# leok7v/sqz

Measured on AMD Instinct MI355X. Metric: encode MB/s + decode MB/s, 32KB window, batched blocks, 1/2/4/8 MI355X, higher is better.
Workload: dtype u8; 1 GPU; 4096 x 262144 B Zipf(s=1) byte blocks, window 2^15, one independent stream per block (BASELINE.json configs[2]); total_blocks=4096, blocks_per_gpu=4096, block_bytes=262144, win_bits=15, parallelism=1 rank; the N>1 runs shard this same batch (strong scaling), finder=index, device=AMD Radeon Graphics (gfx950:sramecc+:xnack-)

## Files before the change

### sqz_amd/csrc/lz77_index.hip

```cpp
#include "sqz_device.h"
#include "sqz_kernels.h"

namespace sqzk {

constexpr int kSharedGiveUp = 8;
constexpr int kXcds = 8;
constexpr int kSortThreads = 1024;
constexpr int kSortWaves = kSortThreads / kWave;

constexpr int kSortTile = 4 * kSortThreads;

constexpr int kSortBins = 1024;
constexpr int kSortCntRow = kSortBins + 2;
struct SortLds {
    uint32_t elem[kSortTile];
    uint16_t dig[kSortTile];
    uint16_t cnt[kSortWaves][kSortCntRow];
    uint32_t gbase[3][kSortBins];
    uint32_t delta[kSortBins];
    uint32_t wtot[kSortWaves];
};

struct __attribute__((packed)) U32u { uint32_t v; };

__device__ __forceinline__ uint32_t load_u32_unaligned(const uint8_t* p) {
    return reinterpret_cast<const U32u*>(p)->v;
}

__device__ __forceinline__ uint64_t peers_of(uint32_t digit, bool valid, int bits) {
    const uint64_t all = __ballot(valid);
    uint32_t lo = (uint32_t)all, hi = (uint32_t)(all >> 32);
#pragma unroll
    for (int bit = 0; bit < 10; bit++) {
        if (bit < bits) {
            const uint32_t mine = (uint32_t)((int32_t)(digit << (31 - bit)) >> 31);
            const uint64_t m = __ballot(mine != 0u);
            lo &= ~((uint32_t)m ^ mine);
            hi &= ~((uint32_t)(m >> 32) ^ mine);
        }
    }
    return ((uint64_t)hi << 32) | lo;
}

__device__ __forceinline__ uint32_t lanes_below(uint64_t mask) {
    return __builtin_amdgcn_mbcnt_hi((uint32_t)(mask >> 32),
                                     __builtin_amdgcn_mbcnt_lo((uint32_t)mask, 0u));
}

__device__ __forceinline__ uint32_t sort_key(const uint8_t* src, uint64_t bytes, uint32_t k) {
    return (uint64_t)k + 4 <= bytes ? (__builtin_bswap32(load_u32_unaligned(src + k)) >> 8)
                                    : (((uint32_t)src[k] << 16) | ((uint32_t)src[k + 1] << 8) | (uint32_t)src[k + 2]);
}

typedef uint32_t __attribute__((may_alias)) SortCntPair;

struct SortSec {
#ifdef SQZ_STATS
    uint64_t t[8] = {0, 0, 0, 0, 0, 0, 0, 0};
    uint64_t last = 0;
#endif
};
#ifdef SQZ_STATS
#define SORT_SEC(s, k) { const uint64_t n_ = __builtin_readcyclecounter(); (s).t[k] += n_ - (s).last; (s).last = n_; }
#define SORT_SEC_LOADS(s, k) { asm volatile("s_waitcnt vmcnt(0)" ::: "memory"); SORT_SEC(s, k) }
#else
#define SORT_SEC(s, k)
#define SORT_SEC_LOADS(s, k)
#endif

template <int kBits, bool kSmall>
__device__ __forceinline__ void sort_pass(SortLds& lds, const int pass, const uint8_t* __restrict__ src,
                                          const uint64_t bytes, const uint32_t count, const bool carry,
                                          const uint32_t* __restrict__ from, uint32_t* __restrict__ to, SortSec& sec) {
    constexpr int kDigits = 1 << kBits;
    constexpr int kTpd = kSortThreads / kDigits;
    constexpr int kWpt = kSortWaves / kTpd;
    const int tid = threadIdx.x;
    const int lane = tid & (kWave - 1);
    const int wave = __builtin_amdgcn_readfirstlane(tid >> 6);
    const bool first = kSmall ? kBits == 10 : pass == 0;
    uint32_t* const gbase = lds.gbase[pass];

    auto fetch = [&](uint32_t tile, uint32_t (&raw)[4]) {
#pragma unroll
        for (int j = 0; j < 4; j++) {
            const uint32_t k = tile + (uint32_t)(wave * 256 + j * kWave + lane);
            if (first) {
                const uint32_t last = (uint32_t)(bytes - 4);
                raw[j] = load_u32_unaligned(src + (k < last ? k : last));
            } else {
                raw[j] = from[k < count ? k : count - 1u];
            }
        }
    };
    auto key_from = [&](uint32_t raw, uint32_t k) {
        const uint32_t be = __builtin_bswap32(raw);
        return (uint64_t)k + 4 <= bytes ? be >> 8 : be & 0x00FFFFFFu;
    };
    auto decode = [&](uint32_t tile, const uint32_t (&raw)[4], uint32_t (&elem)[4], uint32_t (&digit)[4], bool (&valid)[4]) {
#pragma unroll
        for (int j = 0; j < 4; j++) {
            const uint32_t k = tile + (uint32_t)(wave * 256 + j * kWave + lane);
            valid[j] = k < count;
            const uint32_t pos = valid[j] ? (first ? k : raw[j]) : 0u;
            digit[j] = 0; elem[j] = pos;
            if (!valid[j]) { continue; }
            if (kSmall) {
                if (first) {
                    const uint32_t key = key_from(raw[j], k);
                    digit[j] = key & 0x3FFu;
                    elem[j] = pos | ((key >> 10) << 18);
                } else if (pass == 1) {
                    digit[j] = (pos >> 18) & 0x7Fu;
                } else {
                    digit[j] = pos >> 25;
                    elem[j] = pos & 0x3FFFFu;
                }
            } else if (first) {
                digit[j] = key_from(raw[j], k) & 0xFFu;
            } else if (pass == 1) {
                const uint32_t w = (uint32_t)src[pos] | ((uint32_t)src[pos + 1] << 8);
                digit[j] = w >> 8;
                if (carry) { elem[j] = pos | ((w & 0xFFu) << 24); }
            } else {
                digit[j] = carry ? (pos >> 24) : (uint32_t)src[pos];
                if (carry) { elem[j] = pos & 0x00FFFFFFu; }
            }
        }
    };

    uint32_t ahead[4], elem[4], digit[4], wrank[4];
    bool valid[4];
    fetch(0u, ahead);
    decode(0u, ahead, elem, digit, valid);
    SORT_SEC_LOADS(sec, 1)
    for (uint32_t tile = 0; tile < count; tile += (uint32_t)kSortTile) {
        const uint32_t n_tile = count - tile < (uint32_t)kSortTile ? count - tile : (uint32_t)kSortTile;
        fetch(tile + (uint32_t)kSortTile, ahead);
        {
            SortCntPair* const row = reinterpret_cast<SortCntPair*>(lds.cnt[wave]);
            for (int d = lane; d < kDigits / 2; d += kWave) { row[d] = 0u; }
        }
#pragma unroll
        for (int j = 0; j < 4; j++) {
            const uint64_t peers = peers_of(digit[j], valid[j], kBits);
            const uint32_t rank = lanes_below(peers);
            wrank[j] = valid[j] ? (uint32_t)lds.cnt[wave][digit[j]] + rank : 0u;
            __builtin_amdgcn_wave_barrier();
            if (valid[j] && rank == 0) {
                lds.cnt[wave][digit[j]] = (uint16_t)(lds.cnt[wave][digit[j]] + (uint32_t)__builtin_popcountll(peers));
            }
            __builtin_amdgcn_wave_barrier();
        }
        lds_barrier();
        SORT_SEC(sec, 2)
        const int sd = tid / kTpd;
        const int sw = (tid % kTpd) * kWpt;
        uint32_t c[kWpt], sum = 0;
#pragma unroll
        for (int i = 0; i < kWpt; i++) { c[i] = lds.cnt[sw + i][sd]; sum += c[i]; }
        const uint32_t incl = wave_scan(sum);
        if (lane == kWave - 1) { lds.wtot[wave] = incl; }
        lds_barrier();
        SORT_SEC(sec, 3)
        uint32_t at = wave_scan(lane < wave ? lds.wtot[lane] : 0u);
        at = (uint32_t)__builtin_amdgcn_readlane((int)at, kWave - 1) + incl - sum;
        const uint32_t run = at;
#pragma unroll
        for (int i = 0; i < kWpt; i++) { lds.cnt[sw + i][sd] = (uint16_t)at; at += c[i]; }
        const uint32_t run_end = kTpd > 1 ? (uint32_t)__shfl((int)at, lane | (kTpd - 1)) : at;
        if (tid % kTpd == 0) {
            const uint32_t g = gbase[sd];
            lds.delta[sd] = g - run;
            gbase[sd] = g + (run_end - run);
        }
        lds_barrier();
        SORT_SEC(sec, 4)
#pragma unroll
        for (int j = 0; j < 4; j++) {
            if (valid[j]) {
                const uint32_t slot = (uint32_t)lds.cnt[wave][digit[j]] + wrank[j];
                if (slot < (uint32_t)kSortTile) {
                    lds.elem[slot] = elem[j];
                    lds.dig[slot] = (uint16_t)digit[j];
                }
            }
        }
        lds_barrier();
        SORT_SEC(sec, 5)
#pragma unroll
        for (int j = 0; j < 4; j++) {
            const uint32_t slot = (uint32_t)(j * kSortThreads + tid);
            const uint32_t s = slot < n_tile ? slot : n_tile - 1u;
            const uint32_t dest = s + lds.delta[lds.dig[s]];
            to[dest < count ? dest : count - 1u] = lds.elem[s];
        }
        SORT_SEC(sec, 6)
        decode(tile + (uint32_t)kSortTile, ahead, elem, digit, valid);
        SORT_SEC_LOADS(sec, 1)
    }
    __threadfence_block();
    __syncthreads();
}

__global__ __launch_bounds__(kSortThreads)
void index_sort_kernel(const uint8_t* __restrict__ in,
                       const uint64_t* __restrict__ in_off,
                       uint32_t n_blocks,
                       uint32_t* __restrict__ buf_a,
                       uint32_t* __restrict__ buf_b,
                       uint64_t slots) {
    __shared__ SortLds lds;
    const uint32_t b = blockIdx.x;
    if (b >= n_blocks || in_off[b + 1] > slots) { return; }
    const int tid = threadIdx.x;
    const int lane = tid & (kWave - 1);
    const int wave = __builtin_amdgcn_readfirstlane(tid >> 6);

    const uint8_t* src = in + in_off[b];
    const uint64_t bytes = in_off[b + 1] - in_off[b];
    if (bytes < 3) { return; }
    const uint32_t count = (uint32_t)(bytes - 2);
    uint32_t* const pa = buf_a + in_off[b];
    uint32_t* const pb = buf_b + in_off[b];
    if (bytes == 3) {
        if (tid == 0) { pa[0] = 0u; }
        return;
    }
    const bool small = bytes <= (1u << 18);
    const bool carry = bytes <= (1u << 24);
    const int w0 = small ? 10 : 8, w1 = small ? 7 : 8, w2 = small ? 7 : 8;
    const int s1 = w0, s2 = w0 + w1;
    const uint32_t m0 = (1u << w0) - 1u, m1 = (1u << w1) - 1u;
    SortSec sec;
#ifdef SQZ_STATS
    sec.last = __builtin_readcyclecounter();
    const uint64_t sec_begin = sec.last;
#endif
    for (int d = tid; d < 3 * kSortBins; d += kSortThreads) { (&lds.gbase[0][0])[d] = 0; }
    __syncthreads();
    auto count_key = [&](uint32_t key) {
        atomicAdd(&lds.gbase[0][key & m0], 1u);
        atomicAdd(&lds.gbase[1][(key >> s1) & m1], 1u);
        atomicAdd(&lds.gbase[2][key >> s2], 1u);
    };
    const uint32_t quads = bytes >= 8 ? (uint32_t)((bytes - 8) / 4) + 1u : 0u;
    if ((uint32_t)tid < quads) {
        uint32_t lo = load_u32_unaligned(src + 4u * (uint32_t)tid), hi = load_u32_unaligned(src + 4u * (uint32_t)tid + 4u);
        for (uint32_t q = (uint32_t)tid; q < quads; q += (uint32_t)kSortThreads) {
            const uint64_t eight = ((uint64_t)hi << 32) | lo;
            const uint32_t nq = q + (uint32_t)kSortThreads < quads ? q + (uint32_t)kSortThreads : q;
            lo = load_u32_unaligned(src + 4u * nq); hi = load_u32_unaligned(src + 4u * nq + 4u);
#pragma unroll
            for (int j = 0; j < 4; j++) { count_key(__builtin_bswap32((uint32_t)(eight >> (8 * j))) >> 8); }
        }
    }
    for (uint32_t k = 4u * quads + (uint32_t)tid; k < count; k += (uint32_t)kSortThreads) { count_key(sort_key(src, bytes, k)); }
    __syncthreads();
    if (wave < 3) {
        uint32_t* const g = lds.gbase[wave];
        const int per = (1 << (wave == 0 ? w0 : wave == 1 ? w1 : w2)) / kWave;
        uint32_t sum = 0;
        for (int j = 0; j < per; j++) { sum += g[per * lane + j]; }
        uint32_t excl = wave_scan(sum) - sum;
        for (int j = 0; j < per; j++) { const uint32_t v = g[per * lane + j]; g[per * lane + j] = excl; excl += v; }
    }
    __syncthreads();
    SORT_SEC(sec, 0)

    if (small) {
        sort_pass<10, true>(lds, 0, src, bytes, count, carry, pb, pa, sec);
        for (int pass = 1; pass < 3; pass++) {
            sort_pass<7, true>(lds, pass, src, bytes, count, carry, pass == 1 ? pa : pb, pass == 1 ? pb : pa, sec);
        }
    } else {
        for (int pass = 0; pass < 3; pass++) {
            sort_pass<8, false>(lds, pass, src, bytes, count, carry, pass == 1 ? pa : pb, pass == 1 ? pb : pa, sec);
        }
    }
#ifdef SQZ_STATS
    if (tid == 0 && b == 1) {
        printf("sort block 1: cycles %llu: hist %llu; tiles: loads %llu rank %llu scan_a %llu scan_b %llu place %llu copy_out %llu\n",
               (unsigned long long)(sec.last - sec_begin), (unsigned long long)sec.t[0], (unsigned long long)sec.t[1],
               (unsigned long long)sec.t[2], (unsigned long long)sec.t[3], (unsigned long long)sec.t[4],
               (unsigned long long)sec.t[5], (unsigned long long)sec.t[6]);
    }
#endif
}

__global__ __launch_bounds__(256)
void index_match_kernel(const uint8_t* __restrict__ in,
                        const uint64_t* __restrict__ in_off,
                        uint32_t n_blocks, uint32_t window,
                        const uint32_t* __restrict__ sorted,
                        uint32_t* __restrict__ match, uint32_t groups, uint64_t slots) {
    const uint32_t xcd = blockIdx.x % (uint32_t)kXcds;
    const uint32_t local = blockIdx.x / (uint32_t)kXcds;
    const uint32_t b = (local / groups) * (uint32_t)kXcds + xcd;
    const uint32_t group = local % groups;
    if (b >= n_blocks || in_off[b + 1] > slots) { return; }
    const uint8_t* src = in + in_off[b];
    const uint64_t bytes = in_off[b + 1] - in_off[b];
    if (bytes < 3) { return; }
    const uint32_t n = (uint32_t)bytes;
    const uint32_t count = n - 2;
    const uint32_t* S = sorted + in_off[b];
    uint32_t* M = match + in_off[b];

    const int lane = (int)(threadIdx.x & (kWave - 1));
    const uint32_t pages = (count + (uint32_t)kWave - 1u) / (uint32_t)kWave;
    const uint32_t waves = groups * (blockDim.x / (uint32_t)kWave);
    const uint32_t per_wave = (pages + waves - 1u) / waves;
    const uint32_t wave_id = group * (blockDim.x / (uint32_t)kWave) + (threadIdx.x - (uint32_t)lane) / (uint32_t)kWave;
    const uint32_t page_lo = wave_id * per_wave;
    const uint32_t page_hi = page_lo + per_wave < pages ? page_lo + per_wave : pages;
    auto load16 = [&](uint32_t at, uint32_t& w0, uint32_t& w1, uint32_t& w2, uint32_t& w3) {
        if (at + 16 <= n) {
            w0 = load_u32_unaligned(src + at); w1 = load_u32_unaligned(src + at + 4);
            w2 = load_u32_unaligned(src + at + 8); w3 = load_u32_unaligned(src + at + 12);
        } else {
            uint32_t w[4] = {0, 0, 0, 0};
            for (uint32_t k = 0; k < 16 && at + k < n; k++) { w[k >> 2] |= (uint32_t)src[at + k] << (8 * (k & 3)); }
            w0 = w[0]; w1 = w[1]; w2 = w[2]; w3 = w[3];
        }
    };
    uint32_t prev_i = 0, prev0 = 0, prev1 = 0, prev2 = 0, prev3 = 0;
    if (page_lo > 0 && page_lo < page_hi) {
        prev_i = S[(page_lo - 1u) * (uint32_t)kWave + (uint32_t)lane];
        load16(prev_i, prev0, prev1, prev2, prev3);
    }
    for (uint32_t pg = page_lo; pg < page_hi; pg++) {
        const uint32_t r0 = pg * (uint32_t)kWave;
        const bool have_prev = pg > 0;
        const uint32_t r = r0 + (uint32_t)lane;
        const bool valid = r < count;
        const uint32_t i = valid ? S[r] : 0u;
        const uint32_t cap = (n - i) < (uint32_t)kLenMax ? (n - i) : (uint32_t)kLenMax;
        const uint32_t reach = i < window - 1 ? i : window - 1;
        uint32_t own0 = 0, own1 = 0, own2 = 0, own3 = 0;
        if (valid) { load16(i, own0, own1, own2, own3); }
        const uint32_t key = own0 & 0x00FFFFFFu;
        uint32_t best = 0, dist = 0;
        auto walk = [&](uint32_t q_from) {
            if (q_from == 0 || best >= cap) { return; }
            auto inside = [&](uint32_t r) {
                const uint32_t p = S[r];
                if (p + 4 > n) { return false; }
                return (load_u32_unaligned(src + p) & 0x00FFFFFFu) == key && i - p <= reach;
            };
            uint32_t q_lo;
            {
                uint32_t d = 4, bad = 0, good = q_from;
                bool open = true;
                while (open) {
                    if (d >= q_from) { bad = 0; open = false; if (inside(0)) { good = 0; } else { bad = 1; } }
                    else if (inside(q_from - d)) { good = q_from - d; d <<= 1; }
                    else { bad = q_from - d + 1; open = false; }
                }
                uint32_t lo = bad, hi = good;
                while (lo < hi) {
                    const uint32_t mid = lo + ((hi - lo) >> 1);
                    if (inside(mid)) { hi = mid; } else { lo = mid + 1; }
                }
                q_lo = lo;
            }
            uint8_t own_next = best >= (uint32_t)kLenMin ? src[i + best] : (uint8_t)0;
            for (uint32_t q = q_from; q > q_lo && best < cap; ) {
                q--;
                const uint32_t p = S[q];
                if (best >= (uint32_t)kLenMin && src[p + best] != own_next) { continue; }
                uint32_t k = 3;
                while (k < cap) {
                    if (i + k + 4 <= n) {
                        const uint32_t x = load_u32_unaligned(src + p + k) ^ load_u32_unaligned(src + i + k);
                        if (x != 0) { k += (uint32_t)__builtin_ctz(x) >> 3; break; }
                        k += 4;
                    } else {
                        if (src[p + k] != src[i + k]) { break; }
                        k++;
                    }
                }
                if (k > cap) { k = cap; }
                if (k > best) {
                    best = k; dist = i - p;
                    if (best < cap) { own_next = src[i + best]; }
                }
            }
        };
        const uint32_t key0 = (uint32_t)__builtin_amdgcn_readfirstlane((int)key);
        if (__ballot(valid && key == key0 && i + 16 <= n) == ~0ull) {
            bool done = false, deferred = false;
            uint32_t resume = 0;
            uint32_t page_base = r0, page = i, pb0 = own0, pb1 = own1, pb2 = own2, pb3 = own3;
            for (int64_t c = (int64_t)r0 + kWave - 2; c >= 0; c--) {
                if (c < (int64_t)page_base) {
                    page_base -= (uint32_t)kWave;
                    page = S[page_base + (uint32_t)lane];
                    load16(page, pb0, pb1, pb2, pb3);
                }
                const int at = (int)(c - (int64_t)page_base);
                const uint32_t pc = (uint32_t)__builtin_amdgcn_readlane((int)page, at);
                const bool below = (int64_t)r > c;
                const uint32_t d = i - pc;
                if (below && d > reach) { done = true; }
                if (__ballot(!done) == 0) { break; }
                const uint32_t c0 = (uint32_t)__builtin_amdgcn_readlane((int)pb0, at);
                if ((c0 & 0x00FFFFFFu) != key0) { break; }
                const uint32_t c1 = (uint32_t)__builtin_amdgcn_readlane((int)pb1, at);
                const uint32_t c2 = (uint32_t)__builtin_amdgcn_readlane((int)pb2, at);
                const uint32_t c3 = (uint32_t)__builtin_amdgcn_readlane((int)pb3, at);
                const uint32_t x0 = own0 ^ c0, x1 = own1 ^ c1, x2 = own2 ^ c2, x3 = own3 ^ c3;
                uint32_t len = x0 != 0 ? ((uint32_t)__builtin_ctz(x0) >> 3)
                             : x1 != 0 ? 4u + ((uint32_t)__builtin_ctz(x1) >> 3)
                             : x2 != 0 ? 8u + ((uint32_t)__builtin_ctz(x2) >> 3)
                             : x3 != 0 ? 12u + ((uint32_t)__builtin_ctz(x3) >> 3) : 16u;
                const bool want = below && !done;
                if (want && len == 16u && cap > 16u) {
                    deferred = true;
                    resume = (uint32_t)c + 1u;
                    done = true;
                } else {
                    if (len > cap) { len = cap; }
                    if (want && len > best) {
                        best = len; dist = d;
                        if (best >= cap) { done = true; }
                    }
                }
                if (__builtin_popcountll(__ballot(deferred)) >= kSharedGiveUp) {
                    if (!done) {
                        deferred = true;
                        resume = below ? (uint32_t)c : r;
                        done = true;
                    }
                    break;
                }
            }
            if (deferred) { walk(resume); }
            M[i] = best >= (uint32_t)kLenMin ? ((best << 16) | dist) : (key & 0xFFu);
            prev_i = i; prev0 = own0; prev1 = own1; prev2 = own2; prev3 = own3;
            continue;
        }
        bool done = !valid;
        bool later = false;
        uint32_t resume = 0;
        for (int k = 1; k <= kWave; k++) {
            const int from = lane - k;
            const bool in_cur = from >= 0;
            if (!done && !in_cur && !have_prev) { done = true; }
            if (__ballot(!done) == 0) { break; }
            const int addr = (from & (kWave - 1)) << 2;
            uint32_t pc = (uint32_t)__builtin_amdgcn_ds_bpermute(addr, (int)i);
            uint32_t c0 = (uint32_t)__builtin_amdgcn_ds_bpermute(addr, (int)own0);
            uint32_t c1 = (uint32_t)__builtin_amdgcn_ds_bpermute(addr, (int)own1);
            const bool back = __ballot(!done && !in_cur) != 0;
            if (back) {
                const uint32_t qc = (uint32_t)__builtin_amdgcn_ds_bpermute(addr, (int)prev_i);
                const uint32_t q0 = (uint32_t)__builtin_amdgcn_ds_bpermute(addr, (int)prev0);
                const uint32_t q1 = (uint32_t)__builtin_amdgcn_ds_bpermute(addr, (int)prev1);
                pc = in_cur ? pc : qc; c0 = in_cur ? c0 : q0; c1 = in_cur ? c1 : q1;
            }
            const uint32_t x0 = own0 ^ c0, x1 = own1 ^ c1;
            if (!done && (x0 & 0x00FFFFFFu) != 0) { done = true; }
            const uint32_t d = i - pc;
            if (!done && d > reach) { done = true; }
            uint32_t len = x0 != 0 ? ((uint32_t)__builtin_ctz(x0) >> 3) : x1 != 0 ? 4u + ((uint32_t)__builtin_ctz(x1) >> 3) : 8u;
            if (__ballot(!done && len == 8u && cap > 8u) != 0) {
                uint32_t c2 = (uint32_t)__builtin_amdgcn_ds_bpermute(addr, (int)own2);
                uint32_t c3 = (uint32_t)__builtin_amdgcn_ds_bpermute(addr, (int)own3);
                if (back) {
                    const uint32_t q2 = (uint32_t)__builtin_amdgcn_ds_bpermute(addr, (int)prev2);
                    const uint32_t q3 = (uint32_t)__builtin_amdgcn_ds_bpermute(addr, (int)prev3);
                    c2 = in_cur ? c2 : q2; c3 = in_cur ? c3 : q3;
                }
                const uint32_t x2 = own2 ^ c2, x3 = own3 ^ c3;
                if (len == 8u) {
                    len = x2 != 0 ? 8u + ((uint32_t)__builtin_ctz(x2) >> 3) : x3 != 0 ? 12u + ((uint32_t)__builtin_ctz(x3) >> 3) : 16u;
                }
            }
            if (!done) {
                if (len == 16u && cap > 16u) {
                    later = true;
                    resume = r - (uint32_t)k + 1u;
                    done = true;
                } else {
                    if (len > cap) { len = cap; }
                    if (len > best) {
                        best = len; dist = d;
                        if (best >= cap) { done = true; }
                    }
                    if (!done && k == kWave) {
                        later = true;
                        resume = r - (uint32_t)kWave;
                        done = true;
                    }
                }
            }
        }
        if (later) { walk(resume); }
        if (valid) { M[i] = best >= (uint32_t)kLenMin ? ((best << 16) | dist) : (key & 0xFFu); }
        prev_i = i; prev0 = own0; prev1 = own1; prev2 = own2; prev3 = own3;
    }
}

constexpr int kChunk = 32;
constexpr int kTile = kChunk * kWave;
constexpr int kChunkRow = kChunk + 1;

struct ParseLds {
    uint32_t m[kChunkRow * kWave];
};

__device__ __forceinline__ uint32_t parse_slot(uint32_t k) { return k + (k / (uint32_t)kChunk); }

__device__ __forceinline__ uint32_t parse_step(uint32_t w) {
    const uint32_t len = w >> 16;
    return len != 0 ? len : 1u;
}

__global__ __launch_bounds__(kWave)
void index_parse_kernel(const uint8_t* __restrict__ in,
                        const uint64_t* __restrict__ in_off,
                        uint32_t n_blocks,
                        const uint32_t* __restrict__ match,
                        uint32_t* __restrict__ tokens,
                        uint32_t* __restrict__ tok_count, uint64_t slots) {
    __shared__ ParseLds lds;
    const uint32_t b = blockIdx.x;
    if (b >= n_blocks) { return; }
    const int lane = threadIdx.x;
    if (in_off[b + 1] > slots) {
        if (lane == 0) { tok_count[b] = kRefused; }
        return;
    }
    const uint8_t* src = in + in_off[b];
    const uint64_t bytes = in_off[b + 1] - in_off[b];
    const uint32_t* M = match + in_off[b];
    uint32_t* tok = tokens + in_off[b];

    uint32_t ntok = 0;
    uint32_t entry = 0;
    for (uint64_t tile = 0; tile < bytes; tile += (uint64_t)kTile) {
        const uint64_t left = bytes - tile;
        const uint32_t have = left < (uint64_t)kTile ? (uint32_t)left : (uint32_t)kTile;
        if (entry >= have) { entry -= (uint32_t)kTile; continue; }
        __syncthreads();
        for (uint32_t k = lane; k < have; k += kWave) {
            lds.m[parse_slot(k)] = (tile + k + 2 < bytes) ? M[tile + k] : (uint32_t)src[tile + k];
        }
        __syncthreads();

        const uint32_t lo = (uint32_t)lane * (uint32_t)kChunk;
        const uint32_t room = have > lo ? (have - lo < (uint32_t)kChunk ? have - lo : (uint32_t)kChunk) : 0u;
        const uint32_t* row = &lds.m[lane * kChunkRow];
        uint32_t guess = 0;
        uint32_t p = 0;
        while (p < room) {
            guess |= 1u << p;
            const uint32_t w = row[p];
            p += parse_step(w);
        }
        const uint32_t guess_out = lo + p;

        uint32_t mine = 0;
        uint32_t e = entry;
        for (int l = 0; l < kWave; l++) {
            const uint32_t clo = (uint32_t)l * (uint32_t)kChunk;
            if (clo >= have) { break; }
            const uint32_t chi = clo + (uint32_t)kChunk < have ? clo + (uint32_t)kChunk : have;
            if (e >= chi) { continue; }
            const uint32_t g = (uint32_t)__builtin_amdgcn_readlane((int)guess, l);
            const uint32_t gout = (uint32_t)__builtin_amdgcn_readlane((int)guess_out, l);
            uint32_t real = 0;
            uint32_t q = e - clo;
            const uint32_t croom = chi - clo;
            for (;;) {
                if ((g >> q) & 1u) {
                    real |= g & ~((1u << q) - 1u);
                    e = gout;
                    break;
                }
                real |= 1u << q;
                const uint32_t w = (uint32_t)__builtin_amdgcn_readfirstlane((int)lds.m[l * kChunkRow + (int)q]);
                q += parse_step(w);
                if (q >= croom) { e = clo + q; break; }
            }
            if (lane == l) { mine = real; }
        }
        entry = e - (uint32_t)kTile;

        const uint32_t cnt = (uint32_t)__builtin_popcount(mine);
        const uint32_t incl = wave_scan(cnt);
        uint32_t at = ntok + incl - cnt;
        uint32_t bits = mine;
        while (bits != 0) {
            const uint32_t k = (uint32_t)__builtin_ctz(bits);
            bits &= bits - 1u;
            const uint32_t w = row[k];
            tok[at++] = (w >> 16) != 0 ? (kTokMatch | w) : (w & 0xFFu);
        }
        ntok += (uint32_t)__builtin_amdgcn_readlane((int)incl, kWave - 1);
    }
    if (lane == 0) { tok_count[b] = ntok; }
}

void launch_index_sort(const uint8_t* in, const uint64_t* in_off, uint32_t n_blocks,
                       uint32_t* buf_a, uint32_t* buf_b, uint64_t slots,
                       hipStream_t stream) {
    if (n_blocks == 0) { return; }
    hipLaunchKernelGGL(index_sort_kernel, dim3(n_blocks), dim3(kSortThreads), 0, stream,
                       in, in_off, n_blocks, buf_a, buf_b, slots);
}

void launch_index_match(const uint8_t* in, const uint64_t* in_off, uint32_t n_blocks,
                        uint32_t window, const uint32_t* sorted, uint32_t* match,
                        uint32_t match_groups, uint64_t slots, hipStream_t stream) {
    if (n_blocks == 0) { return; }
    if (match_groups < 1) { match_groups = 1; }
    const uint32_t rounded = (n_blocks + (uint32_t)kXcds - 1) / (uint32_t)kXcds * (uint32_t)kXcds;
    while ((uint64_t)match_groups * rounded > 0x7FFFFFFFull) { match_groups = (match_groups + 1) / 2; }
    hipLaunchKernelGGL(index_match_kernel, dim3(rounded * match_groups), dim3(256), 0, stream,
                       in, in_off, n_blocks, window, sorted, match, match_groups, slots);
}

void launch_index_parse(const uint8_t* in, const uint64_t* in_off, uint32_t n_blocks,
                        const uint32_t* match, uint32_t* tokens, uint32_t* tok_count,
                        uint64_t slots, hipStream_t stream) {
    if (n_blocks == 0) { return; }
    hipLaunchKernelGGL(index_parse_kernel, dim3(n_blocks), dim3(kWave), 0, stream,
                       in, in_off, n_blocks, match, tokens, tok_count, slots);
}

}
```

Before: 14320 MB/s.

## Prefetch parse tiles into registers, streamline fixup, and stage token writes via LDS

The LZ77 parse kernel now loads the next tile's match words into registers while the current tile is being parsed, replacing the per-tile synchronous global loads. The serial fixup loop jumps straight from chunk to chunk and merges guessed bits in one pass instead of scanning every lane. Tokens are compacted into LDS and written to global memory as coalesced rows rather than scattered per-lane stores. It also adds optional cycle-counter instrumentation and tightens early exit when the entry runs past the end of a tile. The cost is higher register pressure from the prefetch buffer and the 32-word row copy, plus extra barriers.

Result: faster. 15110 MB/s (median of 6 runs) (+5.5%).

```diff
diff --git a/sqz_amd/csrc/lz77_index.hip b/sqz_amd/csrc/lz77_index.hip
--- a/sqz_amd/csrc/lz77_index.hip
+++ b/sqz_amd/csrc/lz77_index.hip
@@ -517,6 +517,40 @@
     return len != 0 ? len : 1u;
 }
 
+constexpr int kTileRows = kTile / kWave;
+__device__ __forceinline__ void parse_fetch(uint32_t (&w)[kTileRows], const uint32_t* __restrict__ M,
+                                            const uint64_t tile, const uint64_t bytes, const int lane) {
+    const uint64_t left = bytes - tile;
+    const uint32_t last = left < (uint64_t)kTile ? (uint32_t)left - 1u : (uint32_t)kTile - 1u;
+    const uint32_t* __restrict__ T = M + tile;
+#pragma unroll
+    for (int j = 0; j < kTileRows; j++) {
+        const uint32_t k = (uint32_t)(j * kWave + lane);
+        w[j] = T[k < last ? k : last];
+    }
+}
+
+__device__ __forceinline__ uint32_t per_tile(uint32_t v) {
+#ifndef SQZ_WAVE_EMU
+    asm volatile("" : "+v"(v));
+#endif
+    return v;
+}
+
+struct ParseSec {
+#ifdef SQZ_STATS
+    uint64_t t[5] = {0, 0, 0, 0, 0};
+    uint64_t last = 0;
+#endif
+};
+#ifdef SQZ_STATS
+#define PARSE_SEC(s, k) SORT_SEC(s, k)
+#define PARSE_SEC_LOADS(s, k) SORT_SEC_LOADS(s, k)
+#else
+#define PARSE_SEC(s, k)
+#define PARSE_SEC_LOADS(s, k)
+#endif
+
 __global__ __launch_bounds__(kWave)
 void index_parse_kernel(const uint8_t* __restrict__ in,
                         const uint64_t* __restrict__ in_off,
@@ -537,17 +571,38 @@
     const uint32_t* M = match + in_off[b];
     uint32_t* tok = tokens + in_off[b];
 
+    if (bytes == 0) {
+        if (lane == 0) { tok_count[b] = 0; }
+        return;
+    }
+    const uint32_t lit1 = (uint32_t)src[bytes - 1];
+    const uint32_t lit2 = (uint32_t)src[bytes >= 2 ? bytes - 2 : 0];
+
+    ParseSec sec;
+#ifdef SQZ_STATS
+    sec.last = __builtin_readcyclecounter();
+    const uint64_t sec_begin = sec.last;
+#endif
     uint32_t ntok = 0;
     uint32_t entry = 0;
-    for (uint64_t tile = 0; tile < bytes; tile += (uint64_t)kTile) {
+    uint32_t fly[kTileRows];
+    parse_fetch(fly, M, 0, bytes, lane);
+    auto do_tile = [&](const uint64_t tile) __attribute__((always_inline)) -> bool {
         const uint64_t left = bytes - tile;
         const uint32_t have = left < (uint64_t)kTile ? (uint32_t)left : (uint32_t)kTile;
-        if (entry >= have) { entry -= (uint32_t)kTile; continue; }
-        __syncthreads();
-        for (uint32_t k = lane; k < have; k += kWave) {
-            lds.m[parse_slot(k)] = (tile + k + 2 < bytes) ? M[tile + k] : (uint32_t)src[tile + k];
-        }
-        __syncthreads();
+        if (entry >= have) { return false; }
+        PARSE_SEC_LOADS(sec, 0)
+        lds_barrier();
+        const int t2 = left < (uint64_t)(kTile + 2) ? (int)left - 2 : kTile;
+        uint32_t* const mine_at = &lds.m[parse_slot((uint32_t)lane)];
+#pragma unroll
+        for (int j = 0; j < kTileRows; j++) {
+            const int tj = t2 - j * kWave;
+            mine_at[j * (kWave + kWave / kChunk)] = lane < tj ? fly[j] : lane == tj ? lit2 : lit1;
+        }
+        lds_barrier();
+        parse_fetch(fly, M, tile + (uint64_t)kTile < bytes ? tile + (uint64_t)kTile : tile, bytes, lane);
+        PARSE_SEC(sec, 1)
 
         const uint32_t lo = (uint32_t)lane * (uint32_t)kChunk;
         const uint32_t room = have > lo ? (have - lo < (uint32_t)kChunk ? have - lo : (uint32_t)kChunk) : 0u;
@@ -560,47 +615,78 @@
             p += parse_step(w);
         }
         const uint32_t guess_out = lo + p;
-
-        uint32_t mine = 0;
+        PARSE_SEC(sec, 2)
+
+        uint32_t extra = 0;
+        uint32_t from = (uint32_t)kChunk;
         uint32_t e = entry;
-        for (int l = 0; l < kWave; l++) {
-            const uint32_t clo = (uint32_t)l * (uint32_t)kChunk;
-            if (clo >= have) { break; }
-            const uint32_t chi = clo + (uint32_t)kChunk < have ? clo + (uint32_t)kChunk : have;
-            if (e >= chi) { continue; }
-            const uint32_t g = (uint32_t)__builtin_amdgcn_readlane((int)guess, l);
-            const uint32_t gout = (uint32_t)__builtin_amdgcn_readlane((int)guess_out, l);
+        while (e < have) {
+            const uint32_t l = e / (uint32_t)kChunk;
+            const uint32_t clo = l * (uint32_t)kChunk;
+            const uint32_t g = (uint32_t)__builtin_amdgcn_readlane((int)guess, (int)l);
+            uint32_t q = e - clo;
+            if (((g >> q) & 1u) != 0) {
+                e = (uint32_t)__builtin_amdgcn_readlane((int)guess_out, (int)l);
+                if ((uint32_t)lane == l) { from = q; }
+                continue;
+            }
+            const uint32_t croom = have - clo < (uint32_t)kChunk ? have - clo : (uint32_t)kChunk;
             uint32_t real = 0;
-            uint32_t q = e - clo;
-            const uint32_t croom = chi - clo;
-            for (;;) {
-                if ((g >> q) & 1u) {
-                    real |= g & ~((1u << q) - 1u);
-                    e = gout;
-                    break;
-                }
+            do {
                 real |= 1u << q;
-                const uint32_t w = (uint32_t)__builtin_amdgcn_readfirstlane((int)lds.m[l * kChunkRow + (int)q]);
+                const uint32_t w = (uint32_t)__builtin_amdgcn_readfirstlane((int)lds.m[l * kChunkRow + q]);
                 q += parse_step(w);
-                if (q >= croom) { e = clo + q; break; }
-            }
-            if (lane == l) { mine = real; }
-        }
+            } while (q < croom && ((g >> q) & 1u) == 0);
+            const bool met = q < croom;
+            e = met ? (uint32_t)__builtin_amdgcn_readlane((int)guess_out, (int)l) : clo + q;
+            if ((uint32_t)lane == l) { extra = real; from = met ? q : (uint32_t)kChunk; }
+        }
+        const uint32_t mine = extra | (from < (uint32_t)kChunk ? guess & (~0u << from) : 0u);
         entry = e - (uint32_t)kTile;
-
+        PARSE_SEC(sec, 3)
+
+        uint32_t mw[kChunk];
+#pragma unroll
+        for (int j = 0; j < kChunk; j++) { mw[j] = row[j]; }
         const uint32_t cnt = (uint32_t)__builtin_popcount(mine);
         const uint32_t incl = wave_scan(cnt);
-        uint32_t at = ntok + incl - cnt;
-        uint32_t bits = mine;
-        while (bits != 0) {
-            const uint32_t k = (uint32_t)__builtin_ctz(bits);
-            bits &= bits - 1u;
-            const uint32_t w = row[k];
-            tok[at++] = (w >> 16) != 0 ? (kTokMatch | w) : (w & 0xFFu);
-        }
-        ntok += (uint32_t)__builtin_amdgcn_readlane((int)incl, kWave - 1);
+        const uint32_t total = (uint32_t)__builtin_amdgcn_readlane((int)incl, kWave - 1);
+        lds_barrier();
+        uint32_t at = incl - cnt;
+#pragma unroll
+        for (int j = 0; j < kChunk; j++) {
+            if ((mine >> j) & 1u) {
+                lds.m[at++] = (mw[j] >> 16) != 0 ? (kTokMatch | mw[j]) : (mw[j] & 0xFFu);
+            }
+        }
+        lds_barrier();
+        uint32_t* const out = tok + ntok;
+        const uint32_t last = total - 1u;
+        const uint32_t ln = per_tile((uint32_t)lane);
+#pragma unroll
+        for (int j = 0; j < kTileRows; j++) {
+            const uint32_t k = (uint32_t)(j * kWave) + ln;
+            const uint32_t n = (k < last ? k : last) & (uint32_t)(kTile - 1);
+            out[n] = lds.m[n];
+        }
+        ntok += total;
+        PARSE_SEC(sec, 4)
+        return true;
+    };
+    static_assert(kTile > kLenMax, "a token never reaches over a whole tile");
+    if (do_tile(0)) {
+        for (uint64_t tile = (uint64_t)kTile; tile < bytes; tile += (uint64_t)kTile) {
+            if (!do_tile(tile)) { break; }
+        }
     }
     if (lane == 0) { tok_count[b] = ntok; }
+#ifdef SQZ_STATS
+    if (lane == 0 && b == 1) {
+        printf("parse block 1: cycles %llu: tiles: arrived %llu stage %llu guess %llu fixup %llu write %llu\n",
+               (unsigned long long)(sec.last - sec_begin), (unsigned long long)sec.t[0], (unsigned long long)sec.t[1],
+               (unsigned long long)sec.t[2], (unsigned long long)sec.t[3], (unsigned long long)sec.t[4]);
+    }
+#endif
 }
 
 void launch_index_sort(const uint8_t* in, const uint64_t* in_off, uint32_t n_blocks,
```
